# hpcaitech/CachedEmbedding

Measured on AMD Instinct MI355X. Metric: embedding lookups/sec (cache op + EmbeddingBag fwd + bwd/SGD), Criteo-1TB table @1% cache, higher is better.
Workload: dtype f32

## Files before the change

cachedembedding_amd/csrc/ce_bag.hip:

```cpp
#include <stdlib.h>

#include <algorithm>

#include "ce_common.h"

namespace ce {

#ifdef CE_ABLATIONS
#define CE_DBG(x) (x)
#else
#define CE_DBG(x) 0
#endif

struct BagParams {
  const float* weight;
  float* dst;
  const void* grad_out;
  const int64_t* indices;
  const void* offsets;
  const float* psw;
  int64_t nnz;
  int32_t num_bags;
  int32_t rowlen;
  int32_t g_log2;
// ... 305 lines not shown
  return lo;
}

template <typename KT> struct KeyOps;
template <> struct KeyOps<uint32_t> {
  static __device__ __forceinline__ uint32_t make(uint32_t row, int i) { return (row << 10) | (uint32_t)i; }
  static __device__ __forceinline__ uint32_t row(uint32_t k) { return k >> 10; }
  static __device__ __forceinline__ int idx(uint32_t k) { return (int)(k & 1023u); }
  static __device__ __forceinline__ uint32_t invalid() { return 0xffffffffu; }
  static __device__ __forceinline__ uint32_t row_invalid() { return 0x3fffffu; }
};
template <> struct KeyOps<unsigned long long> {
  static __device__ __forceinline__ unsigned long long make(uint32_t row, int i) {
    return ((unsigned long long)row << 32) | (uint32_t)i;
  }
  static __device__ __forceinline__ uint32_t row(unsigned long long k) { return (uint32_t)(k >> 32); }
  static __device__ __forceinline__ int idx(unsigned long long k) { return (int)(uint32_t)k; }
  static __device__ __forceinline__ unsigned long long invalid() { return ~0ull; }
  static __device__ __forceinline__ uint32_t row_invalid() { return 0xffffffffu; }
};

template <typename KT>
__device__ __forceinline__ KT shfl_xor_key(KT v, int m) { return __shfl_xor(v, m); }
template <>
__device__ __forceinline__ unsigned long long shfl_xor_key<unsigned long long>(unsigned long long v, int m) {
  const unsigned lo = __shfl_xor((unsigned)v, m), hi = __shfl_xor((unsigned)(v >> 32), m);
  return ((unsigned long long)hi << 32) | lo;
}

template <typename KT>
__device__ __forceinline__ void tile_sort_1024(KT (&key)[4], KT* lds, int tid) {
  for (int k = 2; k <= kBwdTile; k <<= 1) {
    for (int j = k >> 1; j > 0; j >>= 1) {
      if (j >= 256) {
#pragma unroll
        for (int r = 0; r < 4; ++r) lds[tid * 4 + r] = key[r];
        __syncthreads();
#pragma unroll
        for (int r = 0; r < 4; ++r) {
          const int i = tid * 4 + r;
          const KT other = lds[i ^ j];
          const bool lower = (i & j) == 0, up = (i & k) == 0;
          const KT lo = key[r] < other ? key[r] : other, hi = key[r] < other ? other : key[r];
          key[r] = (lower == up) ? lo : hi;
        }
        __syncthreads();
      } else if (j >= 4) {
#pragma unroll
        for (int r = 0; r < 4; ++r) {
          const int i = tid * 4 + r;
          const KT other = shfl_xor_key<KT>(key[r], j >> 2);
          const bool lower = (i & j) == 0, up = (i & k) == 0;
          const KT lo = key[r] < other ? key[r] : other, hi = key[r] < other ? other : key[r];
          key[r] = (lower == up) ? lo : hi;
        }
      } else {
#pragma unroll
        for (int r = 0; r < 4; ++r) {
          if (r & j) continue;
          const bool up = ((tid * 4 + r) & k) == 0;
          const KT a = key[r], b = key[r | j];
          if ((a > b) == up) {
            key[r] = b;
            key[r | j] = a;
          }
        }
      }
    }
  }
#pragma unroll
  for (int r = 0; r < 4; ++r) lds[tid * 4 + r] = key[r];
  __syncthreads();
}

constexpr int kSegLen = 16384;
constexpr int kSegKeys = 16;
#ifndef CE_SEG_BUCKETS
#define CE_SEG_BUCKETS 8192
#endif
constexpr int kSegBuckets = CE_SEG_BUCKETS;
constexpr int kExclRun = 32;
constexpr unsigned kExclFlag = 0x80000000u;

template <bool SRC, bool EXCL, bool ROWS>
__global__ __launch_bounds__(1024) void k_bag_presort_seg(const int64_t* __restrict__ indices, int64_t nnz_per_batch,
                                                         int32_t segs_per_batch, int64_t n_segs, uint32_t num_rows,
                                                         unsigned long long* __restrict__ keys_out, BagParams lay,
                                                         int64_t off_stride, const int64_t* __restrict__ ids,
                                                         int64_t* __restrict__ ids_minmax, int64_t* slots_io,
                                                         const int32_t* __restrict__ inverted,
                                                         const int* __restrict__ status) {
  __shared__ unsigned long long lk[kSegLen];
  static_assert(sizeof(unsigned long long) * kSegLen <= 160 * 1024 - 1024, "gfx950: 160 KB of LDS per CU");
  int* const cnt = (int*)lk;
  __shared__ int wsum[16];
  __shared__ long long mm_s[2][16];
  const int tid = threadIdx.x, lane = tid & 63, wv = tid >> 6;
  for (int64_t seg = blockIdx.x; seg < n_segs; seg += gridDim.x) {
    const int64_t batch = seg / segs_per_batch;
    const int sib = (int)(seg - batch * segs_per_batch);
    const int64_t in_base = batch * nnz_per_batch + (int64_t)sib * kSegLen;
    const int64_t base = seg * kSegLen;
    const int n_here = (int)min((int64_t)kSegLen, nnz_per_batch - (int64_t)sib * kSegLen);
    BagParams q = lay;
    if (SRC && lay.offsets) q.offsets = (const char*)lay.offsets + batch * off_stride * (lay.off64 ? 8 : 4);
    for (int i = tid; i <= kSegBuckets; i += 1024) cnt[i] = 0;
    __syncthreads();
    unsigned long long key[kSegKeys];
    int place[kSegKeys], bkt[kSegKeys];
    int32_t slot_r[ROWS ? kSegKeys : 1];
    if (ROWS) {
      const bool failed = *status != CE_OK;
      int32_t row_r[kSegKeys];
#pragma unroll
      for (int r = 0; r < kSegKeys; ++r) {
        const int e = r * 1024 + tid;
        row_r[r] = e < n_here ? (int32_t)slots_io[in_base + e] : -1;
      }
#pragma unroll
      for (int r = 0; r < kSegKeys; ++r) slot_r[r] = (row_r[r] >= 0 && !failed) ? inverted[row_r[r]] : -1;
#pragma unroll
      for (int r = 0; r < kSegKeys; ++r) {
        const int e = r * 1024 + tid;
        if (e < n_here) slots_io[in_base + e] = (int64_t)slot_r[r];
      }
    }
#pragma unroll
    for (int r = 0; r < kSegKeys; ++r) {
      const int e = r * 1024 + tid;
      key[r] = ~0ull;
      bkt[r] = kSegBuckets;
      if (e < n_here) {
        const int64_t row = ROWS ? (int64_t)slot_r[ROWS ? r : 0] : indices[in_base + e];
        const bool valid = (uint64_t)row < (uint64_t)num_rows;
        if (valid || SRC) {
          unsigned low = (unsigned)e;
          if (SRC && !(CE_DBG(lay.debug) & 2))
            low = (unsigned)out_row(q, lay.offsets ? find_bag(q, sib * kSegLen + e) : sib * kSegLen + e);
          key[r] = ((unsigned long long)(valid ? (uint32_t)row : 0xffffffffu) << 32) | low;
          if (valid) bkt[r] = (int)(row & (kSegBuckets - 1));
        }
      }
      if (CE_DBG(lay.debug) & 8) {
        place[r] = 0;
        continue;
      }
      const int b0 = __builtin_amdgcn_readfirstlane(bkt[r]);
      if (__all(bkt[r] == b0)) {
        int first = 0;
        if (lane == 0) first = atomicAdd(&cnt[b0], 64);
        place[r] = __shfl(first, 0) + lane;
      } else {
        place[r] = atomicAdd(&cnt[bkt[r]], 1);
      }
    }
    __syncthreads();
    constexpr int kPer = kSegBuckets / 1024;
    int c4[kPer], sum = 0;
#pragma unroll
    for (int q = 0; q < kPer; ++q) { c4[q] = cnt[tid * kPer + q]; sum += c4[q]; }
    int inc = sum;
#pragma unroll
    for (int d = 1; d < 64; d <<= 1) {
      const int o = __shfl_up(inc, d);
      if (lane >= d) inc += o;
    }
    if (lane == 63) wsum[wv] = inc;
    __syncthreads();
    int pre = inc - sum;
    for (int k = 0; k < wv; ++k) pre += wsum[k];
    int total = 0;
    for (int k = 0; k < 16; ++k) total += wsum[k];
#pragma unroll
    for (int q = 0; q < kPer; ++q) { cnt[tid * kPer + q] = pre; pre += c4[q]; }
    if (tid == 0) cnt[kSegBuckets] = total;
    __syncthreads();
    if (!EXCL) {
      int pos[kSegKeys];
#pragma unroll
      for (int r = 0; r < kSegKeys; ++r) pos[r] = cnt[bkt[r]] + place[r];
      __syncthreads();
#pragma unroll
      for (int r = 0; r < kSegKeys; ++r) lk[pos[r]] = key[r];
      __syncthreads();
#pragma unroll
      for (int r = 0; r < kSegKeys; ++r) keys_out[base + r * 1024 + tid] = lk[r * 1024 + tid];
      __syncthreads();
      continue;
    }
    int pos[kSegKeys];
#pragma unroll
    for (int r = 0; r < kSegKeys; ++r) pos[r] = cnt[bkt[r]] + place[r];
    __syncthreads();
#pragma unroll
    for (int r = 0; r < kSegKeys; ++r) lk[pos[r]] = key[r];
    __syncthreads();
    {
      const uint32_t* hi = (const uint32_t*)lk;
      const int p0 = tid * kSegKeys;
      for (int p = p0; p < p0 + kSegKeys; ++p) {
        const uint32_t row = hi[2 * p + 1];
        if (row == 0xffffffffu) break;
        const uint32_t b = row & (kSegBuckets - 1);
        if (p > 0 && (hi[2 * p - 1] & (kSegBuckets - 1)) == b && hi[2 * p - 1] != 0xffffffffu) continue;
        int e = p + 1;
        while (e < kSegLen && e - p <= kExclRun && hi[2 * e + 1] != 0xffffffffu && (hi[2 * e + 1] & (kSegBuckets - 1)) == b) ++e;
        if (e - p > kExclRun) continue;
        for (int i = p + 1; i < e; ++i) {
          const unsigned long long k = lk[i];
          int j = i;
          while (j > p && (uint32_t)(lk[j - 1] >> 32) > (uint32_t)(k >> 32)) { lk[j] = lk[j - 1]; --j; }
          lk[j] = k;
        }
        for (int a = p; a < e;) {
          int z = a + 1;
          while (z < e && (uint32_t)(lk[z] >> 32) == (uint32_t)(lk[a] >> 32)) ++z;
          if ((a >> 4) == ((z - 1) >> 4)) lk[a] |= kExclFlag;
          a = z;
        }
      }
    }
    __syncthreads();
#pragma unroll
    for (int r = 0; r < kSegKeys; ++r) keys_out[base + r * 1024 + tid] = lk[r * 1024 + tid];
    if (ids_minmax) {
      long long lo = INT64_MAX, hi2 = INT64_MIN;
      if (ids) {
#pragma unroll
        for (int r = 0; r < kSegKeys; ++r) {
          const int e = r * 1024 + tid;
          if (e < n_here) {
            const long long v = ids[in_base + e];
            lo = v < lo ? v : lo;
            hi2 = v > hi2 ? v : hi2;
          }
        }
      } else {
        lo = INT64_MIN; hi2 = INT64_MAX;
      }
#pragma unroll
      for (int d = 32; d >= 1; d >>= 1) {
        const long long ol = __shfl_xor(lo, d), oh = __shfl_xor(hi2, d);
        lo = ol < lo ? ol : lo;
        hi2 = oh > hi2 ? oh : hi2;
      }
      if (lane == 0) { mm_s[0][wv] = lo; mm_s[1][wv] = hi2; }
      __syncthreads();
      if (tid == 0) {
        for (int k = 1; k < 16; ++k) {
          lo = mm_s[0][k] < lo ? mm_s[0][k] : lo;
          hi2 = mm_s[1][k] > hi2 ? mm_s[1][k] : hi2;
        }
        ids_minmax[2 * seg] = lo;
        ids_minmax[2 * seg + 1] = hi2;
      }
    }
    __syncthreads();
  }
}

template <typename VT, int NCH, typename KT, int R, typename AT>
__global__ __launch_bounds__(256) void k_bag_bwd_tile(BagParams p) {
  using K = KeyOps<KT>;
  using A = Act<AT, VT>;
  __shared__ KT keys[kBwdTile];
  __shared__ int bagl[kBwdTile];
  __shared__ float scl[kBwdTile];

  const int tid = threadIdx.x;
  const int G = 1 << p.g_log2;
  const int ngroups = 256 >> p.g_log2;
  const int grp = tid >> p.g_log2;
  const int gl = tid & (G - 1);
  const int rowlen = p.rowlen;
  const int dim = rowlen * (int)(sizeof(VT) / 4);
  const typename A::V* __restrict__ GO = (const typename A::V*)p.grad_out;
  const int tile_len = p.tile_len;
  const int64_t total = p.presorted ? ((p.nnz + kSegLen - 1) / kSegLen) * kSegLen : p.nnz;
  const int ntiles = (int)((total + tile_len - 1) / tile_len);

  for (int tile = blockIdx.x; tile < ntiles; tile += gridDim.x) {
    const int j0 = tile * tile_len;
    const int nv = min(tile_len, (int)(total - j0));
    const bool presorted = p.presorted != nullptr;
    KT kr[4];
#pragma unroll
    for (int r = 0; r < 4; ++r) {
      const int i = tid * 4 + r;
      kr[r] = K::invalid();
      int j = j0 + i;
      uint32_t row = 0xffffffffu;
      if (presorted) {
        const unsigned long long sk = i < nv ? p.presorted[(int64_t)j0 + i] : ~0ull;
        j = -1;
        if (sk != ~0ull) {
          row = (uint32_t)(sk >> 32);
          j = (int)((((int64_t)j0 + i) / kSegLen) * kSegLen) + (int)(uint32_t)sk;
        }
      } else if (i < nv) {
        const int64_t r64 = p.indices[j];
        if ((uint64_t)r64 < (uint64_t)p.num_rows) row = (uint32_t)r64;
      } else {
        j = -1;
      }
      if (j >= 0) {
        const int bag = find_bag(p, j);
        float sc = p.alpha;
        if (p.psw) sc *= p.psw[j];
        if (p.mode == CE_MODE_MEAN) {
          const int len = bag_end(p, bag) - ld_off(p, bag);
          if (len > 1) sc = sc / (float)len;
        }
        bagl[i] = (int)out_row(p, bag);
        scl[i] = sc;
        if (row != 0xffffffffu) kr[r] = K::make(row, i);
      }
    }
    if (CE_DBG(p.debug) == 3) { __syncthreads(); continue; }
    if (presorted) {
#pragma unroll
      for (int r = 0; r < 4; ++r) keys[tid * 4 + r] = kr[r];
      __syncthreads();
    } else {
      tile_sort_1024<KT>(kr, keys, tid);
    }
    if (CE_DBG(p.debug) == 4) continue;
    const int kChunk = (nv + ngroups - 1) / ngroups;
    const int nchunks = (nv + kChunk - 1) / kChunk;
    for (int ck = grp; ck < nchunks; ck += ngroups) {
      const int s0 = ck * kChunk, s1 = min(nv, s0 + kChunk);
      VT acc[NCH];
#pragma unroll
      for (int c = 0; c < NCH; ++c) acc[c] = vzero<VT>();
      uint32_t cur = K::row(keys[s0]);
      for (int q = s0; q < s1; q += R) {
        VT v[R][NCH];
        float sc[R];
        uint32_t rw[R];
#pragma unroll
        for (int t = 0; t < R; ++t) {
          const KT key = (q + t < s1) ? keys[q + t] : K::invalid();
          const bool on = key != K::invalid();
          const int li = on ? K::idx(key) : 0;
          rw[t] = on ? K::row(key) : K::row_invalid();
          sc[t] = on ? scl[li] : 0.f;
          const int64_t orow = bagl[li];
#pragma unroll
          for (int c = 0; c < NCH; ++c) {
            const int ch = gl + c * G;
            v[t][c] = vzero<VT>();
            if (on && ch < rowlen) v[t][c] = A::up(__builtin_nontemporal_load(&GO[orow * rowlen + ch]));
          }
        }
        __builtin_amdgcn_s_waitcnt(0x0F70);
#pragma unroll
        for (int t = 0; t < R; ++t) {
          if (rw[t] != K::row_invalid()) {
            if (rw[t] != cur) {
#pragma unroll
              for (int c = 0; c < NCH; ++c) {
                if (cur != K::row_invalid())
                  flush_chunk(p.dst + (int64_t)cur * dim, acc[c], gl, G, c, rowlen, CE_DBG(p.debug));
                acc[c] = vzero<VT>();
              }
              cur = rw[t];
            }
#pragma unroll
            for (int c = 0; c < NCH; ++c) acc[c] = acc[c] + v[t][c] * sc[t];
          }
        }
      }
#pragma unroll
      for (int c = 0; c < NCH; ++c) {
        if (cur != K::row_invalid()) flush_chunk(p.dst + (int64_t)cur * dim, acc[c], gl, G, c, rowlen, CE_DBG(p.debug));
      }
    }
    __syncthreads();
  }
}

template <typename VT, int NCH, int R, bool NTG, bool EXCL, typename AT, bool PAIR = false>
__global__ __launch_bounds__(256) void k_bag_bwd_stream(BagParams p, int64_t total, const long long* __restrict__ seg_ranges) {
  using A = Act<AT, VT>;
  static_assert(!PAIR || (sizeof(typename A::V) == 8 && R % 2 == 0), "PAIR: 4 x 16 bit per lane, keys two at a time");
  __shared__ unsigned long long lk[256 * (R > 4 ? R : 4)];
  const int tid = threadIdx.x;
  const int G = 1 << p.g_log2;
  const int ngroups = 256 >> p.g_log2;
  const int grp = tid >> p.g_log2;
  const int gl = tid & (G - 1);
  const int rowlen = p.rowlen;
  const int dim = rowlen * (int)(sizeof(VT) / 4);
  const typename A::V* __restrict__ GO = (const typename A::V*)p.grad_out;
  const VT* __restrict__ WV = (const VT*)p.dst;
  const unsigned long long* __restrict__ keys = p.presorted;
  bool excl = false;
  if (EXCL) {
    const int nseg = (int)(total / kSegLen);
    int clash = nseg > 64 || seg_ranges == nullptr;
    if (!clash) {
      for (int pr = tid; pr < nseg * nseg; pr += 256) {
        const int a = pr / nseg, b2 = pr - a * nseg;
        if (a >= b2) continue;
        const long long alo = seg_ranges[2 * a], ahi = seg_ranges[2 * a + 1];
        const long long blo = seg_ranges[2 * b2], bhi = seg_ranges[2 * b2 + 1];
        if (alo <= ahi && blo <= bhi && !(ahi < blo || bhi < alo)) clash = 1;
      }
    }
    excl = __syncthreads_or(clash) == 0;
  }
  const int64_t all_groups = (int64_t)gridDim.x * ngroups;
  const int64_t round = R > 16 ? R : 16;
  const int64_t share = ((total + all_groups - 1) / all_groups + round - 1) / round * round;
  const int64_t s0 = share_of(p, grp, ngroups) * share;
  const int64_t s1 = min(total, s0 + share);
  if (s0 >= s1) return;
  const float alpha = p.alpha;
  const int kc = 4 * G > R ? 4 * G : R;
  unsigned long long* mylk = lk + grp * kc;
  VT acc[NCH];
#pragma unroll
  for (int c = 0; c < NCH; ++c) acc[c] = vzero<VT>();
  uint32_t cur = 0xffffffffu;
  bool cur_excl = false;
  for (int64_t c0 = s0; c0 < s1; c0 += kc) {
    for (int k = gl; k < kc; k += G) mylk[k] = c0 + k < s1 ? keys[c0 + k] : ~0ull;
    const int64_t c1 = min(s1, c0 + kc);
    for (int64_t q = c0; q < c1; q += R) {
      VT v[R][NCH];
      VT w2[EXCL ? R : 1][NCH];
      u32x4 raw[PAIR ? R / 2 : 1][NCH];
      uint32_t rw[R];
      uint32_t heads = 0;
#pragma unroll
      for (int t = 0; t < R; ++t) {
        const unsigned long long k = mylk[(int)(q - c0) + t];
        const bool on = k != ~0ull && (uint32_t)(k >> 32) < p.num_rows;
        rw[t] = on ? (uint32_t)(k >> 32) : 0xffffffffu;
        const uint32_t low = (uint32_t)k;
        const int64_t src = (int64_t)(low & ~kExclFlag);
        const bool head = EXCL && excl && on && (low & kExclFlag);
        if (head) heads |= 1u << t;
        if constexpr (PAIR) if (!(t & 1)) {
          const unsigned long long k1 = mylk[(int)(q - c0) + t + 1];
          const bool on1 = k1 != ~0ull && (uint32_t)(k1 >> 32) < p.num_rows;
          const bool mine = (gl & 1) ? on1 : on;
          const int64_t msrc = (gl & 1) ? (int64_t)((uint32_t)k1 & ~kExclFlag) : src;
#pragma unroll
          for (int c = 0; c < NCH; ++c) {
            const int ch = gl + c * G;
            raw[PAIR ? t / 2 : 0][c] = u32x4{0u, 0u, 0u, 0u};
            if (mine && ch < rowlen)
              raw[PAIR ? t / 2 : 0][c] = __builtin_nontemporal_load((const u32x4*)p.grad_out + ((msrc * rowlen + ch) >> 1));
          }
        }
#pragma unroll
        for (int c = 0; c < NCH; ++c) {
          const int ch = gl + c * G;
          v[t][c] = vzero<VT>();
          if (!PAIR && on && ch < rowlen)
            v[t][c] = A::up(NTG ? __builtin_nontemporal_load(&GO[src * rowlen + ch]) : GO[src * rowlen + ch]);
          if (EXCL) {
            w2[t][c] = vzero<VT>();
            if (head && ch < rowlen) w2[t][c] = WV[(int64_t)rw[t] * rowlen + ch];
          }
        }
      }
      __builtin_amdgcn_s_waitcnt(0x0F70);
      if constexpr (PAIR) {
#pragma unroll
        for (int t = 0; t < R; t += 2) {
#pragma unroll
          for (int c = 0; c < NCH; ++c) {
            const u32x4 r = raw[PAIR ? t / 2 : 0][c];
            const u32x2 lo{r.x, r.y}, hi{r.z, r.w};
            const bool odd = gl & 1;
            const u32x2 got = swap_with_pair(odd ? lo : hi);
            v[t][c] = A::up(__builtin_bit_cast(typename A::V, odd ? got : lo));
            v[t + 1][c] = A::up(__builtin_bit_cast(typename A::V, odd ? hi : got));
          }
        }
      }
#pragma unroll
      for (int t = 0; t < R; ++t) {
        if (rw[t] != 0xffffffffu) {
          const bool head = EXCL && ((heads >> t) & 1);
          if (rw[t] != cur || head) {
#pragma unroll
            for (int c = 0; c < NCH; ++c) {
              if (cur != 0xffffffffu) {
                if (EXCL && cur_excl) {
                  const int ch = gl + c * G;
                  if (ch < rowlen) ((VT*)(p.dst + (int64_t)cur * dim))[ch] = acc[c];
                } else {
                  flush_chunk(p.dst + (int64_t)cur * dim, acc[c], gl, G, c, rowlen, CE_DBG(p.debug));
                }
              }
              acc[c] = EXCL ? w2[EXCL ? t : 0][c] : vzero<VT>();
            }
            cur = rw[t];
            cur_excl = head;
          }
#pragma unroll
          for (int c = 0; c < NCH; ++c) acc[c] = acc[c] + v[t][c] * alpha;
        }
      }
    }
  }
  if (cur != 0xffffffffu) {
#pragma unroll
    for (int c = 0; c < NCH; ++c) {
      if (EXCL && cur_excl) {
        const int ch = gl + c * G;
        if (ch < rowlen) ((VT*)(p.dst + (int64_t)cur * dim))[ch] = acc[c];
      } else {
        flush_chunk(p.dst + (int64_t)cur * dim, acc[c], gl, G, c, rowlen, CE_DBG(p.debug));
      }
    }
  }
}

template <typename VT, int NCH, int R, int NTS, typename AT, bool PAIR = false>
__global__ __launch_bounds__(256, 4) void k_bag_fwd_keys(BagParams p, int64_t total) {
  using A = Act<AT, VT>;
  static_assert(!PAIR || (sizeof(typename A::V) == 8 && R % 2 == 0), "PAIR: 4 x 16 bit per lane, keys two at a time");
  __shared__ unsigned long long lk[256 * (R > 4 ? R : 4)];
  const int tid = threadIdx.x;
  const int G = 1 << p.g_log2;
  const int ngroups = 256 >> p.g_log2;
  const int grp = tid >> p.g_log2;
  const int gl = tid & (G - 1);
  const int rowlen = p.rowlen;
  const VT* __restrict__ W = (const VT*)p.weight;
  typename A::V* __restrict__ O = (typename A::V*)p.dst;
  const unsigned long long* __restrict__ keys = p.presorted;
  const int64_t all_groups = (int64_t)gridDim.x * ngroups;
  const int64_t round = R > 16 ? R : 16;
  const int64_t share = ((total + all_groups - 1) / all_groups + round - 1) / round * round;
  const int64_t s0 = share_of(p, grp, ngroups) * share;
  const int64_t s1 = min(total, s0 + share);
  if (s0 >= s1) return;
  const int kc = 4 * G > R ? 4 * G : R;
  unsigned long long* mylk = lk + grp * kc;
  VT prev[NCH];
#pragma unroll
  for (int c = 0; c < NCH; ++c) prev[c] = vzero<VT>();
  uint32_t prev_row = 0xffffffffu;
  for (int64_t c0 = s0; c0 < s1; c0 += kc) {
    for (int k = gl; k < kc; k += G) mylk[k] = c0 + k < s1 ? keys[c0 + k] : ~0ull;
    const int64_t c1 = min(s1, c0 + kc);
    for (int64_t q = c0; q < c1; q += R) {
      VT v[R][NCH];
      uint32_t heads = 0;
      uint32_t last = prev_row;
#pragma unroll
      for (int t = 0; t < R; ++t) {
        const unsigned long long k = mylk[(int)(q - c0) + t];
        const bool on = k != ~0ull;
        const uint32_t rw = (uint32_t)(k >> 32);
        const bool head = on && rw != last;
        if (on) last = rw;
        if (head) heads |= 1u << t;
#pragma unroll
        for (int c = 0; c < NCH; ++c) {
          const int ch = gl + c * G;
          v[t][c] = vzero<VT>();
          if (head && ch < rowlen && rw < p.num_rows) v[t][c] = W[(int64_t)rw * rowlen + ch];
        }
      }
      __builtin_amdgcn_s_waitcnt(0x0F70);
      if constexpr (PAIR) {
        const bool odd = gl & 1;
#pragma unroll
        for (int t = 0; t < R; t += 2) {
          const unsigned long long k0 = mylk[(int)(q - c0) + t], k1 = mylk[(int)(q - c0) + t + 1];
          if (k0 == ~0ull && k1 == ~0ull) continue;
          u32x2 r0[NCH], r1[NCH];
          if ((heads >> t) & 1) {
#pragma unroll
            for (int c = 0; c < NCH; ++c) prev[c] = v[t][c];
          }
#pragma unroll
          for (int c = 0; c < NCH; ++c) r0[c] = __builtin_bit_cast(u32x2, A::down(prev[c]));
          if ((heads >> (t + 1)) & 1) {
#pragma unroll
            for (int c = 0; c < NCH; ++c) prev[c] = v[t + 1][c];
          }
#pragma unroll
          for (int c = 0; c < NCH; ++c) r1[c] = __builtin_bit_cast(u32x2, A::down(prev[c]));
          const unsigned long long km = odd ? k1 : k0;
          const int64_t orow = (int64_t)((uint32_t)km & ~kExclFlag);
#pragma unroll
          for (int c = 0; c < NCH; ++c) {
            const int ch = gl + c * G;
            const u32x2 got = swap_with_pair(odd ? r0[c] : r1[c]);
            const u32x4 o = odd ? u32x4{got.x, got.y, r1[c].x, r1[c].y} : u32x4{r0[c].x, r0[c].y, got.x, got.y};
            if (km != ~0ull && ch < rowlen) store_out<NTS>((u32x4*)p.dst + ((orow * rowlen + ch) >> 1), o);
          }
        }
        prev_row = last;
        continue;
      }
#pragma unroll
      for (int t = 0; t < R; ++t) {
        const unsigned long long k = mylk[(int)(q - c0) + t];
        if (k == ~0ull) continue;
        if ((heads >> t) & 1) {
#pragma unroll
          for (int c = 0; c < NCH; ++c) prev[c] = v[t][c];
// ... 268 lines not shown
static int backward_sgd_impl(float* weight, int64_t num_rows, int32_t dim, const int64_t* indices, int64_t nnz,
                             const void* offsets, int32_t offsets_are_i64, int64_t num_bags,
                             int32_t include_last_offset, const float* per_sample_weights, int32_t mode,
                             int64_t hook_features, const void* grad_out, int act, float lr,
                             const unsigned long long* presorted, ce_stream_t stream) {
  CE_REQUIRE_ACT(act);
  if (num_bags == 0 || nnz == 0) return CE_OK;
  CE_REQUIRE(weight && grad_out && offsets && indices, CE_ERR_INVALID, "null pointer");
  BagParams p{};
  bool vec;
  int nch;
  int rc = fill_params(p, dim, indices, nnz, offsets, offsets_are_i64, num_bags, include_last_offset,
                       per_sample_weights, mode, hook_features, &vec, &nch, weight, act32(grad_out, act), nullptr,
                       act16(grad_out, act));
  if (rc) return rc;
  p.dst = weight;
  p.grad_out = grad_out;
  p.alpha = -lr;
  CE_REQUIRE(num_rows > 0 && num_rows < (int64_t)INT32_MAX, CE_ERR_INVALID, "num_rows out of range");
  p.num_rows = (uint32_t)num_rows;
  p.presorted = presorted;
  return launch_bwd_scatter(p, vec, nch, act, (hipStream_t)stream);
}

extern "C" int ce_bag_backward_sgd(float* weight, int64_t num_rows, int32_t dim, const int64_t* indices,
                                   int64_t nnz, const void* offsets, int32_t offsets_are_i64, int64_t num_bags,
                                   int32_t include_last_offset, const float* per_sample_weights, int32_t mode,
                                   int64_t hook_features, const float* grad_out, float lr, ce_stream_t stream) {
  return backward_sgd_impl(weight, num_rows, dim, indices, nnz, offsets, offsets_are_i64, num_bags,
                           include_last_offset, per_sample_weights, mode, hook_features, grad_out, CE_ACT_F32, lr, nullptr,
                           stream);
}

extern "C" int ce_bag_backward_sgd_act(float* weight, int64_t num_rows, int32_t dim, const int64_t* indices,
                                       int64_t nnz, const void* offsets, int32_t offsets_are_i64, int64_t num_bags,
                                       int32_t include_last_offset, const float* per_sample_weights, int32_t mode,
                                       int64_t hook_features, const void* grad_out, int32_t act_dtype, float lr,
                                       const uint64_t* presorted_keys, ce_stream_t stream) {
  return backward_sgd_impl(weight, num_rows, dim, indices, nnz, offsets, offsets_are_i64, num_bags,
                           include_last_offset, per_sample_weights, mode, hook_features, grad_out, act_dtype, lr,
                           (const unsigned long long*)presorted_keys, stream);
}

extern "C" int ce_bag_backward_sgd_presorted(float* weight, int64_t num_rows, int32_t dim, const int64_t* indices,
                                             int64_t nnz, const void* offsets, int32_t offsets_are_i64,
                                             int64_t num_bags, int32_t include_last_offset,
                                             const float* per_sample_weights, int32_t mode, int64_t hook_features,
                                             const float* grad_out, float lr, const uint64_t* presorted_keys,
                                             ce_stream_t stream) {
  CE_REQUIRE(presorted_keys, CE_ERR_INVALID, "null presorted_keys");
  return backward_sgd_impl(weight, num_rows, dim, indices, nnz, offsets, offsets_are_i64, num_bags,
                           include_last_offset, per_sample_weights, mode, hook_features, grad_out, CE_ACT_F32, lr,
                           (const unsigned long long*)presorted_keys, stream);
}

static int launch_bwd_stream(float* dst, int64_t num_rows, int32_t dim, int64_t nnz, const void* grad_out, int act,
                             float alpha, const unsigned long long* keys, const int64_t* seg_ranges, hipStream_t s) {
  CE_REQUIRE_ACT(act);
  if (nnz == 0) return CE_OK;
  CE_REQUIRE(dst && grad_out && keys, CE_ERR_INVALID, "null pointer");
  CE_REQUIRE(num_rows > 0 && num_rows < (int64_t)INT32_MAX, CE_ERR_INVALID, "num_rows out of range");
  BagParams p{};
  bool vec;
  int nch;
  int rc = fill_params(p, dim, nullptr, nnz, nullptr, 0, 0, 1, nullptr, CE_MODE_SUM, 0, &vec, &nch, dst,
                       act32(grad_out, act), nullptr, act16(grad_out, act));
  if (rc) return rc;
  p.dst = dst;
  p.grad_out = grad_out;
  p.alpha = alpha;
  p.num_rows = (uint32_t)num_rows;
  p.presorted = keys;
#ifdef CE_ABLATIONS
  { const char* dbg = getenv("CE_BWD_DEBUG"); p.debug = dbg ? atoi(dbg) : 0; }
#endif
  p.interleave = 1;
  const int64_t total = cdiv(nnz, kSegLen) * kSegLen;
  constexpr int per_cu = 6;
  const int ngroups = 256 >> p.g_log2;
  const int grid = (int)std::max<int64_t>(1, std::min<int64_t>((int64_t)kNumCU * per_cu, cdiv(total, (int64_t)ngroups * 16)));
  dim3 g(grid), b(256);
  const long long* rg = (const long long*)seg_ranges;
  const bool excl = seg_ranges != nullptr && vec && nch == 1;
#define CE_BWS(VT, N, R, EX) CE_ACT(act, hipLaunchKernelGGL((k_bag_bwd_stream<VT, N, R, true, EX, AT>), g, b, 0, s, p, total, rg))
#define CE_BWS2(N, R, EX)                                                                                              \
  do {                                                                                                                 \
    if (act == CE_ACT_BF16)                                                                                            \
      hipLaunchKernelGGL((k_bag_bwd_stream<f32x4, N, R, true, EX, bf16_t, true>), g, b, 0, s, p, total, rg);           \
    else                                                                                                               \
      hipLaunchKernelGGL((k_bag_bwd_stream<f32x4, N, R, true, EX, f16_t, true>), g, b, 0, s, p, total, rg);            \
  } while (0)
  if (vec && pair16(act, dim, grad_out)) {
    if (nch == 1 && excl) CE_BWS2(1, 16, true);
    else if (nch == 1) CE_BWS2(1, 16, false);
    else if (nch == 2) CE_BWS2(2, 8, false);
    else CE_BWS2(4, 4, false);
  } else if (vec) {
    if (nch == 1 && excl) CE_BWS(f32x4, 1, 16, true);
    else if (nch == 1) CE_BWS(f32x4, 1, 16, false);
    else if (nch == 2) CE_BWS(f32x4, 2, 8, false);
    else CE_BWS(f32x4, 4, 4, false);
  } else {
    if (nch == 1) CE_BWS(float, 1, 16, false);
    else if (nch == 2) CE_BWS(float, 2, 8, false);
    else CE_BWS(float, 4, 4, false);
  }
#undef CE_BWS
#undef CE_BWS2
  CE_LAUNCH_CHECK();
  return CE_OK;
}

extern "C" int ce_bag_backward_sgd_presorted_src(float* weight, int64_t num_rows, int32_t dim, int64_t nnz,
                                                 const float* grad_out, float lr, const uint64_t* src_keys,
                                                 ce_stream_t stream) {
  return launch_bwd_stream(weight, num_rows, dim, nnz, grad_out, CE_ACT_F32, -lr, (const unsigned long long*)src_keys,
                           nullptr, (hipStream_t)stream);
}

extern "C" int ce_bag_backward_sgd_presorted_src_excl(float* weight, int64_t num_rows, int32_t dim, int64_t nnz,
                                                      const float* grad_out, float lr, const uint64_t* src_keys,
                                                      const int64_t* seg_id_ranges, ce_stream_t stream) {
  return launch_bwd_stream(weight, num_rows, dim, nnz, grad_out, CE_ACT_F32, -lr, (const unsigned long long*)src_keys,
                           seg_id_ranges, (hipStream_t)stream);
}

extern "C" int ce_bag_backward_sgd_src_act(float* weight, int64_t num_rows, int32_t dim, int64_t nnz,
                                           const void* grad_out, int32_t act_dtype, float lr, const uint64_t* src_keys,
                                           const int64_t* seg_id_ranges, ce_stream_t stream) {
  return launch_bwd_stream(weight, num_rows, dim, nnz, grad_out, act_dtype, -lr, (const unsigned long long*)src_keys,
                           seg_id_ranges, (hipStream_t)stream);
}

extern "C" int ce_bag_backward_dense_src_act(float* grad_weight, int64_t num_rows, int32_t dim, int64_t nnz,
                                             const void* grad_out, int32_t act_dtype, const uint64_t* src_keys,
                                             ce_stream_t stream) {
  return launch_bwd_stream(grad_weight, num_rows, dim, nnz, grad_out, act_dtype, 1.f,
                           (const unsigned long long*)src_keys, nullptr, (hipStream_t)stream);
}

extern "C" int ce_bag_backward_dense_presorted_src(float* grad_weight, int64_t num_rows, int32_t dim, int64_t nnz,
                                                   const float* grad_out, const uint64_t* src_keys,
                                                   ce_stream_t stream) {
  return launch_bwd_stream(grad_weight, num_rows, dim, nnz, grad_out, CE_ACT_F32, 1.f,
                           (const unsigned long long*)src_keys, nullptr, (hipStream_t)stream);
}

extern "C" int ce_bag_forward_src_keys_act(const float* weight, int64_t num_rows, int32_t dim, int64_t nnz,
                                           const uint64_t* src_keys, void* out, int32_t act_dtype, ce_stream_t stream) {
  CE_REQUIRE_ACT(act_dtype);
  if (nnz == 0) return CE_OK;
  CE_REQUIRE(weight && src_keys && out, CE_ERR_INVALID, "null pointer");
  CE_REQUIRE(num_rows > 0 && num_rows < (int64_t)INT32_MAX, CE_ERR_INVALID, "num_rows out of range");
  BagParams p{};
  bool vec;
  int nch;
  int rc = fill_params(p, dim, nullptr, nnz, nullptr, 0, 0, 1, nullptr, CE_MODE_SUM, 0, &vec, &nch, weight,
                       act32(out, act_dtype), nullptr, act16(out, act_dtype));
  if (rc) return rc;
  p.weight = weight;
  p.dst = (float*)out;
  p.num_rows = (uint32_t)num_rows;
  p.presorted = (const unsigned long long*)src_keys;
  p.interleave = 0;
  const int64_t total = cdiv(nnz, kSegLen) * kSegLen;
  constexpr int per_cu = 16;
  const int ngroups = 256 >> p.g_log2;
  const int grid = (int)std::max<int64_t>(1, std::min<int64_t>((int64_t)kNumCU * per_cu, cdiv(total, (int64_t)ngroups * 16)));
  dim3 g(grid), b(256);
  hipStream_t s = (hipStream_t)stream;
#define CE_FWK(VT, N, R) CE_ACT(act_dtype, hipLaunchKernelGGL((k_bag_fwd_keys<VT, N, R, 1, AT>), g, b, 0, s, p, total))
#define CE_FWK2(N, R)                                                                                     \
  do {                                                                                                    \
    if (act_dtype == CE_ACT_BF16)                                                                         \
      hipLaunchKernelGGL((k_bag_fwd_keys<f32x4, N, R, 1, bf16_t, true>), g, b, 0, s, p, total);           \
    else                                                                                                  \
      hipLaunchKernelGGL((k_bag_fwd_keys<f32x4, N, R, 1, f16_t, true>), g, b, 0, s, p, total);            \
  } while (0)
  if (vec && pair16(act_dtype, dim, out)) {
    if (nch == 1) CE_FWK2(1, 16);
    else if (nch == 2) CE_FWK2(2, 8); else CE_FWK2(4, 4);
  } else if (vec) {
    if (nch == 1) CE_FWK(f32x4, 1, 16);
    else if (nch == 2) CE_FWK(f32x4, 2, 8); else CE_FWK(f32x4, 4, 4);
  } else {
    if (nch == 1) CE_FWK(float, 1, 16); else if (nch == 2) CE_FWK(float, 2, 8); else CE_FWK(float, 4, 4);
  }
#undef CE_FWK
#undef CE_FWK2
  CE_LAUNCH_CHECK();
  return CE_OK;
}

extern "C" int ce_bag_forward_src_keys(const float* weight, int64_t num_rows, int32_t dim, int64_t nnz,
                                       const uint64_t* src_keys, float* out, ce_stream_t stream) {
  return ce_bag_forward_src_keys_act(weight, num_rows, dim, nnz, src_keys, out, CE_ACT_F32, stream);
}

extern "C" int64_t ce_bag_presort_len(int64_t nnz) { return nnz <= 0 ? 0 : cdiv(nnz, kSegLen) * kSegLen; }

static int presort_window_impl(const int64_t* indices, int64_t nnz_per_batch, int64_t n_batches, int64_t num_rows,
                               uint64_t* keys_out, const BagParams* lay, int64_t off_stride, const int64_t* ids,
                               int64_t* ids_minmax, ce_stream_t stream) {
  if (nnz_per_batch == 0 || n_batches == 0) return CE_OK;
  CE_REQUIRE(indices && keys_out && nnz_per_batch > 0 && n_batches > 0, CE_ERR_INVALID, "bad arguments");
  CE_REQUIRE(nnz_per_batch < (int64_t)INT32_MAX - kSegLen, CE_ERR_INVALID, "batch too large");
  CE_REQUIRE(num_rows > 0 && num_rows < (int64_t)INT32_MAX, CE_ERR_INVALID, "num_rows out of range");
  const int64_t spb = cdiv(nnz_per_batch, kSegLen);
  const int64_t nseg = spb * n_batches;
  CE_REQUIRE(spb < (int64_t)INT32_MAX && nseg < (int64_t)INT32_MAX, CE_ERR_INVALID, "too many segments");
  const dim3 grid((unsigned)std::min<int64_t>(nseg, kMaxBlocks)), block(1024);
  int64_t* const no_io = nullptr;
  const int32_t* const no_inv = nullptr;
  const int* const no_st = nullptr;
  if (lay && ids_minmax)
    hipLaunchKernelGGL((k_bag_presort_seg<true, true, false>), grid, block, 0, (hipStream_t)stream, indices, nnz_per_batch,
                       (int32_t)spb, nseg, (uint32_t)num_rows, (unsigned long long*)keys_out, *lay, off_stride, ids,
                       ids_minmax, no_io, no_inv, no_st);
  else if (lay)
    hipLaunchKernelGGL((k_bag_presort_seg<true, false, false>), grid, block, 0, (hipStream_t)stream, indices, nnz_per_batch,
                       (int32_t)spb, nseg, (uint32_t)num_rows, (unsigned long long*)keys_out, *lay, off_stride,
                       (const int64_t*)nullptr, (int64_t*)nullptr, no_io, no_inv, no_st);
  else
    hipLaunchKernelGGL((k_bag_presort_seg<false, false, false>), grid, block, 0, (hipStream_t)stream, indices, nnz_per_batch,
                       (int32_t)spb, nseg, (uint32_t)num_rows, (unsigned long long*)keys_out, BagParams{}, 0ll,
                       (const int64_t*)nullptr, (int64_t*)nullptr, no_io, no_inv, no_st);
  CE_LAUNCH_CHECK();
  return CE_OK;
}

namespace ce {
int presort_window_from_rows(int64_t* slots_io, int64_t nnz_per_batch, int64_t n_batches, int64_t num_rows,
                             const int32_t* inverted, const int* status, int32_t src_keys, const void* offsets,
                             int32_t offsets_are_i64, int64_t offsets_batch_stride, int64_t num_bags,
                             int32_t include_last_offset, int64_t hook_features, uint64_t* keys_out, hipStream_t stream) {
  if (nnz_per_batch == 0 || n_batches == 0) return CE_OK;
  CE_REQUIRE(slots_io && keys_out && inverted && status && nnz_per_batch > 0 && n_batches > 0, CE_ERR_INVALID, "bad arguments");
  CE_REQUIRE(nnz_per_batch < (int64_t)INT32_MAX - kSegLen, CE_ERR_INVALID, "batch too large");
  CE_REQUIRE(num_rows > 0 && num_rows < (int64_t)INT32_MAX, CE_ERR_INVALID, "num_rows out of range");
  const int64_t spb = cdiv(nnz_per_batch, kSegLen);
  const int64_t nseg = spb * n_batches;
  CE_REQUIRE(spb < (int64_t)INT32_MAX && nseg < (int64_t)INT32_MAX, CE_ERR_INVALID, "too many segments");
  const dim3 grid((unsigned)std::min<int64_t>(nseg, kMaxBlocks)), block(1024);
  if (src_keys) {
    CE_REQUIRE(num_bags > 0 && offsets_batch_stride >= 0, CE_ERR_INVALID, "bad offsets");
    CE_REQUIRE(offsets || num_bags == nnz_per_batch, CE_ERR_INVALID,
               "offsets may only be NULL for the one-id-per-bag layout (num_bags == nnz_per_batch)");
    BagParams lay{};
    bool vec;
    int nch;
    int rc = fill_params(lay, 4, nullptr, nnz_per_batch, offsets, offsets_are_i64, num_bags, include_last_offset, nullptr,
                         CE_MODE_SUM, hook_features, &vec, &nch, nullptr, nullptr, nullptr);
    if (rc) return rc;
    hipLaunchKernelGGL((k_bag_presort_seg<true, false, true>), grid, block, 0, stream, (const int64_t*)nullptr,
                       nnz_per_batch, (int32_t)spb, nseg, (uint32_t)num_rows, (unsigned long long*)keys_out, lay,
                       offsets_batch_stride, (const int64_t*)nullptr, (int64_t*)nullptr, slots_io, inverted, status);
  } else {
    hipLaunchKernelGGL((k_bag_presort_seg<false, false, true>), grid, block, 0, stream, (const int64_t*)nullptr,
                       nnz_per_batch, (int32_t)spb, nseg, (uint32_t)num_rows, (unsigned long long*)keys_out, BagParams{},
                       0ll, (const int64_t*)nullptr, (int64_t*)nullptr, slots_io, inverted, status);
  }
  CE_LAUNCH_CHECK();
  return CE_OK;
}
}

extern "C" int ce_bag_presort_window(const int64_t* indices, int64_t nnz_per_batch, int64_t n_batches,
                                     int64_t num_rows, uint64_t* keys_out, ce_stream_t stream) {
  return presort_window_impl(indices, nnz_per_batch, n_batches, num_rows, keys_out, nullptr, 0, nullptr, nullptr, stream);
}

static int presort_window_src_impl(const int64_t* indices, int64_t nnz_per_batch, int64_t n_batches, int64_t num_rows,
                                   const void* offsets, int32_t offsets_are_i64, int64_t offsets_batch_stride,
                                   int64_t num_bags, int32_t include_last_offset, int64_t hook_features,
                                   const int64_t* ids, uint64_t* keys_out, int64_t* seg_id_ranges, ce_stream_t stream) {
  if (nnz_per_batch == 0 || n_batches == 0) return CE_OK;
  CE_REQUIRE(num_bags > 0 && offsets_batch_stride >= 0, CE_ERR_INVALID, "bad offsets");
  CE_REQUIRE(offsets || num_bags == nnz_per_batch, CE_ERR_INVALID,
             "offsets may only be NULL for the one-id-per-bag layout (num_bags == nnz_per_batch)");
  BagParams lay{};
  bool vec;
  int nch;
  int rc = fill_params(lay, 4, indices, nnz_per_batch, offsets, offsets_are_i64, num_bags, include_last_offset,
                       nullptr, CE_MODE_SUM, hook_features, &vec, &nch, nullptr, nullptr, nullptr);
  if (rc) return rc;
#ifdef CE_ABLATIONS
  { const char* dbg = getenv("CE_PRESORT_DEBUG"); lay.debug = dbg ? atoi(dbg) : 0; }
#endif
  return presort_window_impl(indices, nnz_per_batch, n_batches, num_rows, keys_out, &lay, offsets_batch_stride, ids,
                             seg_id_ranges, stream);
}

extern "C" int ce_bag_presort_window_src(const int64_t* indices, int64_t nnz_per_batch, int64_t n_batches,
                                         int64_t num_rows, const void* offsets, int32_t offsets_are_i64,
                                         int64_t offsets_batch_stride, int64_t num_bags, int32_t include_last_offset,
                                         int64_t hook_features, uint64_t* keys_out, ce_stream_t stream) {
  return presort_window_src_impl(indices, nnz_per_batch, n_batches, num_rows, offsets, offsets_are_i64,
                                 offsets_batch_stride, num_bags, include_last_offset, hook_features, nullptr, keys_out,
                                 nullptr, stream);
}

extern "C" int ce_bag_presort_window_src_excl(const int64_t* indices, int64_t nnz_per_batch, int64_t n_batches,
                                              int64_t num_rows, const void* offsets, int32_t offsets_are_i64,
                                              int64_t offsets_batch_stride, int64_t num_bags,
                                              int32_t include_last_offset, int64_t hook_features, const int64_t* ids,
                                              uint64_t* keys_out, int64_t* seg_id_ranges, ce_stream_t stream) {
  CE_REQUIRE(seg_id_ranges, CE_ERR_INVALID, "null seg_id_ranges");
  return presort_window_src_impl(indices, nnz_per_batch, n_batches, num_rows, offsets, offsets_are_i64,
                                 offsets_batch_stride, num_bags, include_last_offset, hook_features, ids, keys_out,
                                 seg_id_ranges, stream);
}

extern "C" int ce_bag_presort(const int64_t* indices, int64_t nnz, int64_t num_rows, uint64_t* keys_out,
                              ce_stream_t stream) {
  return ce_bag_presort_window(indices, nnz, 1, num_rows, keys_out, stream);
}

extern "C" int ce_rows_axpy(float* weight, int64_t num_rows, int32_t dim, const int64_t* index, int64_t n,
                            const float* src_rows, float alpha, ce_stream_t stream) {
  if (n == 0) return CE_OK;
  CE_REQUIRE(weight && index && src_rows, CE_ERR_INVALID, "null pointer");
  CE_REQUIRE(dim > 0 && n > 0 && n < (int64_t)INT32_MAX, CE_ERR_INVALID, "bad sizes");
  CE_REQUIRE(num_rows > 0 && num_rows < (int64_t)INT32_MAX, CE_ERR_INVALID, "num_rows out of range");
  auto al16 = [](const void* q) { return (((uintptr_t)q) & 15) == 0; };
  const bool vec = (dim % 4 == 0) && al16(weight) && al16(src_rows);
  const int rowlen = vec ? dim / 4 : dim;
  int g = 1, gl2 = 0;
  while (g < rowlen && g < 64) { g <<= 1; ++gl2; }
  const int need = (rowlen + g - 1) / g;
  int nch = 1;
  while (nch < need) nch <<= 1;
  CE_REQUIRE(nch <= 4, CE_ERR_UNSUPPORTED, "embedding dim %d too large for this build", dim);
  const int u = nch == 1 ? 8 : (nch == 2 ? 4 : 2);
  const int64_t per_block = (int64_t)(64 / g) * u * 4;
  dim3 grid(grid_for(n, (int)per_block)), block(256);
  hipStream_t s = (hipStream_t)stream;
#define CE_AXPY(VT, N)                                                                                      \
  hipLaunchKernelGGL((k_rows_axpy<VT, N>), grid, block, 0, s, weight, (uint32_t)num_rows, index, n,         \
                     (const VT*)src_rows, rowlen, gl2, dim, alpha)
  if (vec) {
    if (nch == 1) CE_AXPY(f32x4, 1); else if (nch == 2) CE_AXPY(f32x4, 2); else CE_AXPY(f32x4, 4);
  } else {
    if (nch == 1) CE_AXPY(float, 1); else if (nch == 2) CE_AXPY(float, 2); else CE_AXPY(float, 4);
// ... 24 lines not shown
```

Baseline: 3.273 billion.

## Replace LDS-staged segment presort with two-sweep count/scatter kernel; size key LDS dynamically

After: 3.241 billion. Within noise of the previous version (-1.0%).

```diff
diff --git a/cachedembedding_amd/csrc/ce_bag.hip b/cachedembedding_amd/csrc/ce_bag.hip
--- a/cachedembedding_amd/csrc/ce_bag.hip
+++ b/cachedembedding_amd/csrc/ce_bag.hip
@@ -411,14 +411,38 @@
 constexpr int kExclRun = 32;
 constexpr unsigned kExclFlag = 0x80000000u;
 
-template <bool SRC, bool EXCL, bool ROWS>
+__device__ __forceinline__ void seg_scan_counters(int* cnt, int* wsum, int tid) {
+  const int lane = tid & 63, wv = tid >> 6;
+  __syncthreads();
+  constexpr int kPer = kSegBuckets / 1024;
+  int c4[kPer], sum = 0;
+#pragma unroll
+  for (int q = 0; q < kPer; ++q) { c4[q] = cnt[tid * kPer + q]; sum += c4[q]; }
+  int inc = sum;
+#pragma unroll
+  for (int d = 1; d < 64; d <<= 1) {
+    const int o = __shfl_up(inc, d);
+    if (lane >= d) inc += o;
+  }
+  if (lane == 63) wsum[wv] = inc;
+  __syncthreads();
+  int pre = inc - sum;
+  for (int k = 0; k < wv; ++k) pre += wsum[k];
+  int total = 0;
+  for (int k = 0; k < 16; ++k) total += wsum[k];
+#pragma unroll
+  for (int q = 0; q < kPer; ++q) { cnt[tid * kPer + q] = pre; pre += c4[q]; }
+  if (tid == 0) cnt[kSegBuckets] = total;
+  __syncthreads();
+}
+
+template <bool SRC, bool EXCL>
 __global__ __launch_bounds__(1024) void k_bag_presort_seg(const int64_t* __restrict__ indices, int64_t nnz_per_batch,
                                                          int32_t segs_per_batch, int64_t n_segs, uint32_t num_rows,
                                                          unsigned long long* __restrict__ keys_out, BagParams lay,
                                                          int64_t off_stride, const int64_t* __restrict__ ids,
-                                                         int64_t* __restrict__ ids_minmax, int64_t* slots_io,
-                                                         const int32_t* __restrict__ inverted,
-                                                         const int* __restrict__ status) {
+                                                         int64_t* __restrict__ ids_minmax) {
+  static_assert(SRC && EXCL, "the forms without owner-exclusive runs are k_bag_presort_2sweep");
   __shared__ unsigned long long lk[kSegLen];
   static_assert(sizeof(unsigned long long) * kSegLen <= 160 * 1024 - 1024, "gfx950: 160 KB of LDS per CU");
   int* const cnt = (int*)lk;
@@ -437,30 +461,13 @@
     __syncthreads();
     unsigned long long key[kSegKeys];
     int place[kSegKeys], bkt[kSegKeys];
-    int32_t slot_r[ROWS ? kSegKeys : 1];
-    if (ROWS) {
-      const bool failed = *status != CE_OK;
-      int32_t row_r[kSegKeys];
-#pragma unroll
-      for (int r = 0; r < kSegKeys; ++r) {
-        const int e = r * 1024 + tid;
-        row_r[r] = e < n_here ? (int32_t)slots_io[in_base + e] : -1;
-      }
-#pragma unroll
-      for (int r = 0; r < kSegKeys; ++r) slot_r[r] = (row_r[r] >= 0 && !failed) ? inverted[row_r[r]] : -1;
-#pragma unroll
-      for (int r = 0; r < kSegKeys; ++r) {
-        const int e = r * 1024 + tid;
-        if (e < n_here) slots_io[in_base + e] = (int64_t)slot_r[r];
-      }
-    }
 #pragma unroll
     for (int r = 0; r < kSegKeys; ++r) {
       const int e = r * 1024 + tid;
       key[r] = ~0ull;
       bkt[r] = kSegBuckets;
       if (e < n_here) {
-        const int64_t row = ROWS ? (int64_t)slot_r[ROWS ? r : 0] : indices[in_base + e];
+        const int64_t row = indices[in_base + e];
         const bool valid = (uint64_t)row < (uint64_t)num_rows;
         if (valid || SRC) {
           unsigned low = (unsigned)e;
@@ -483,40 +490,7 @@
         place[r] = atomicAdd(&cnt[bkt[r]], 1);
       }
     }
-    __syncthreads();
-    constexpr int kPer = kSegBuckets / 1024;
-    int c4[kPer], sum = 0;
-#pragma unroll
-    for (int q = 0; q < kPer; ++q) { c4[q] = cnt[tid * kPer + q]; sum += c4[q]; }
-    int inc = sum;
-#pragma unroll
-    for (int d = 1; d < 64; d <<= 1) {
-      const int o = __shfl_up(inc, d);
-      if (lane >= d) inc += o;
-    }
-    if (lane == 63) wsum[wv] = inc;
-    __syncthreads();
-    int pre = inc - sum;
-    for (int k = 0; k < wv; ++k) pre += wsum[k];
-    int total = 0;
-    for (int k = 0; k < 16; ++k) total += wsum[k];
-#pragma unroll
-    for (int q = 0; q < kPer; ++q) { cnt[tid * kPer + q] = pre; pre += c4[q]; }
-    if (tid == 0) cnt[kSegBuckets] = total;
-    __syncthreads();
-    if (!EXCL) {
-      int pos[kSegKeys];
-#pragma unroll
-      for (int r = 0; r < kSegKeys; ++r) pos[r] = cnt[bkt[r]] + place[r];
-      __syncthreads();
-#pragma unroll
-      for (int r = 0; r < kSegKeys; ++r) lk[pos[r]] = key[r];
-      __syncthreads();
-#pragma unroll
-      for (int r = 0; r < kSegKeys; ++r) keys_out[base + r * 1024 + tid] = lk[r * 1024 + tid];
-      __syncthreads();
-      continue;
-    }
+    seg_scan_counters(cnt, wsum, tid);
     int pos[kSegKeys];
 #pragma unroll
     for (int r = 0; r < kSegKeys; ++r) pos[r] = cnt[bkt[r]] + place[r];
@@ -588,6 +562,97 @@
   }
 }
 
+constexpr int kSweep = 4;
+template <bool SRC, bool ROWS>
+__global__ __launch_bounds__(1024) __attribute__((amdgpu_waves_per_eu(7))) void k_bag_presort_2sweep(const int64_t* __restrict__ indices, int64_t nnz_per_batch,
+                                                            int32_t segs_per_batch, int64_t n_segs, uint32_t num_rows,
+                                                            unsigned long long* __restrict__ keys_out, BagParams lay,
+                                                            int64_t off_stride, int64_t* slots_io,
+                                                            const int32_t* __restrict__ inverted,
+                                                            const int* __restrict__ status) {
+  __shared__ int cnt[kSegBuckets + 1];
+  __shared__ int wsum[16];
+  static_assert(kSegKeys % kSweep == 0, "whole sweeps");
+  const int tid = threadIdx.x, lane = tid & 63;
+  const int64_t* const src = ROWS ? slots_io : indices;
+  for (int64_t seg = blockIdx.x; seg < n_segs; seg += gridDim.x) {
+    const int64_t batch = seg / segs_per_batch;
+    const int sib = (int)(seg - batch * segs_per_batch);
+    const int64_t in_base = batch * nnz_per_batch + (int64_t)sib * kSegLen;
+    const int64_t base = seg * kSegLen;
+    const int n_here = (int)min((int64_t)kSegLen, nnz_per_batch - (int64_t)sib * kSegLen);
+    BagParams q = lay;
+    if (SRC && lay.offsets) q.offsets = (const char*)lay.offsets + batch * off_stride * (lay.off64 ? 8 : 4);
+    for (int i = tid; i <= kSegBuckets; i += 1024) cnt[i] = 0;
+    __syncthreads();
+    const bool failed = ROWS && *status != CE_OK;
+    for (int r0 = 0; r0 < kSegKeys; r0 += kSweep) {
+      uint32_t row[kSweep];
+#pragma unroll
+      for (int u = 0; u < kSweep; ++u) {
+        const int e = (r0 + u) * 1024 + tid;
+        const int64_t v = e < n_here ? src[in_base + e] : -1;
+        row[u] = ROWS ? (uint32_t)v : ((uint64_t)v < (uint64_t)num_rows ? (uint32_t)v : 0xffffffffu);
+      }
+      if (ROWS) {
+        int32_t slot[kSweep];
+#pragma unroll
+        for (int u = 0; u < kSweep; ++u) slot[u] = ((int32_t)row[u] >= 0 && !failed) ? inverted[(int32_t)row[u]] : -1;
+#pragma unroll
+        for (int u = 0; u < kSweep; ++u) {
+          const int e = (r0 + u) * 1024 + tid;
+          if (e < n_here) slots_io[in_base + e] = (int64_t)slot[u];
+          row[u] = (uint32_t)slot[u] < num_rows ? (uint32_t)slot[u] : 0xffffffffu;
+        }
+      }
+#pragma unroll
+      for (int u = 0; u < kSweep; ++u) {
+        const int bkt = row[u] != 0xffffffffu ? (int)(row[u] & (kSegBuckets - 1)) : kSegBuckets;
+        const int b0 = __builtin_amdgcn_readfirstlane(bkt);
+        if (__all(bkt == b0)) {
+          if (lane == 0) atomicAdd(&cnt[b0], 64);
+        } else {
+          atomicAdd(&cnt[bkt], 1);
+        }
+      }
+    }
+    seg_scan_counters(cnt, wsum, tid);
+    for (int r0 = 0; r0 < kSegKeys; r0 += kSweep) {
+      uint32_t row[kSweep];
+#pragma unroll
+      for (int u = 0; u < kSweep; ++u) {
+        const int e = (r0 + u) * 1024 + tid;
+        const int64_t v = e < n_here ? src[in_base + e] : -1;
+        row[u] = (uint64_t)v < (uint64_t)num_rows ? (uint32_t)v : 0xffffffffu;
+      }
+#pragma unroll
+      for (int u = 0; u < kSweep; ++u) {
+        const int e = (r0 + u) * 1024 + tid;
+        const bool valid = row[u] != 0xffffffffu;
+        unsigned long long key = ~0ull;
+        if (e < n_here && (valid || SRC)) {
+          unsigned low = (unsigned)e;
+          if (SRC && !(CE_DBG(lay.debug) & 2))
+            low = (unsigned)out_row(q, lay.offsets ? find_bag(q, sib * kSegLen + e) : sib * kSegLen + e);
+          key = ((unsigned long long)row[u] << 32) | low;
+        }
+        const int bkt = valid ? (int)(row[u] & (kSegBuckets - 1)) : kSegBuckets;
+        int pos;
+        const int b0 = __builtin_amdgcn_readfirstlane(bkt);
+        if (__all(bkt == b0)) {
+          int first = 0;
+          if (lane == 0) first = atomicAdd(&cnt[b0], 64);
+          pos = __shfl(first, 0) + lane;
+        } else {
+          pos = atomicAdd(&cnt[bkt], 1);
+        }
+        keys_out[base + pos] = key;
+      }
+    }
+    __syncthreads();
+  }
+}
+
 template <typename VT, int NCH, typename KT, int R, typename AT>
 __global__ __launch_bounds__(256) void k_bag_bwd_tile(BagParams p) {
   using K = KeyOps<KT>;
@@ -708,11 +773,16 @@
   }
 }
 
+static inline unsigned key_slice_bytes(int g_log2, int R) {
+  const int G = 1 << g_log2, kc = 4 * G > R ? 4 * G : R;
+  return (unsigned)((256 >> g_log2) * kc * sizeof(unsigned long long));
+}
+
 template <typename VT, int NCH, int R, bool NTG, bool EXCL, typename AT, bool PAIR = false>
 __global__ __launch_bounds__(256) void k_bag_bwd_stream(BagParams p, int64_t total, const long long* __restrict__ seg_ranges) {
   using A = Act<AT, VT>;
   static_assert(!PAIR || (sizeof(typename A::V) == 8 && R % 2 == 0), "PAIR: 4 x 16 bit per lane, keys two at a time");
-  __shared__ unsigned long long lk[256 * (R > 4 ? R : 4)];
+  extern __shared__ unsigned long long lk[];
   const int tid = threadIdx.x;
   const int G = 1 << p.g_log2;
   const int ngroups = 256 >> p.g_log2;
@@ -853,7 +923,7 @@
 __global__ __launch_bounds__(256, 4) void k_bag_fwd_keys(BagParams p, int64_t total) {
   using A = Act<AT, VT>;
   static_assert(!PAIR || (sizeof(typename A::V) == 8 && R % 2 == 0), "PAIR: 4 x 16 bit per lane, keys two at a time");
-  __shared__ unsigned long long lk[256 * (R > 4 ? R : 4)];
+  extern __shared__ unsigned long long lk[];
   const int tid = threadIdx.x;
   const int G = 1 << p.g_log2;
   const int ngroups = 256 >> p.g_log2;
@@ -1288,13 +1358,14 @@
   dim3 g(grid), b(256);
   const long long* rg = (const long long*)seg_ranges;
   const bool excl = seg_ranges != nullptr && vec && nch == 1;
-#define CE_BWS(VT, N, R, EX) CE_ACT(act, hipLaunchKernelGGL((k_bag_bwd_stream<VT, N, R, true, EX, AT>), g, b, 0, s, p, total, rg))
+#define CE_BWS(VT, N, R, EX) \
+  CE_ACT(act, hipLaunchKernelGGL((k_bag_bwd_stream<VT, N, R, true, EX, AT>), g, b, key_slice_bytes(p.g_log2, R), s, p, total, rg))
 #define CE_BWS2(N, R, EX)                                                                                              \
   do {                                                                                                                 \
     if (act == CE_ACT_BF16)                                                                                            \
-      hipLaunchKernelGGL((k_bag_bwd_stream<f32x4, N, R, true, EX, bf16_t, true>), g, b, 0, s, p, total, rg);           \
+      hipLaunchKernelGGL((k_bag_bwd_stream<f32x4, N, R, true, EX, bf16_t, true>), g, b, key_slice_bytes(p.g_log2, R), s, p, total, rg); \
     else                                                                                                               \
-      hipLaunchKernelGGL((k_bag_bwd_stream<f32x4, N, R, true, EX, f16_t, true>), g, b, 0, s, p, total, rg);            \
+      hipLaunchKernelGGL((k_bag_bwd_stream<f32x4, N, R, true, EX, f16_t, true>), g, b, key_slice_bytes(p.g_log2, R), s, p, total, rg); \
   } while (0)
   if (vec && pair16(act, dim, grad_out)) {
     if (nch == 1 && excl) CE_BWS2(1, 16, true);
@@ -1375,13 +1446,14 @@
   const int grid = (int)std::max<int64_t>(1, std::min<int64_t>((int64_t)kNumCU * per_cu, cdiv(total, (int64_t)ngroups * 16)));
   dim3 g(grid), b(256);
   hipStream_t s = (hipStream_t)stream;
-#define CE_FWK(VT, N, R) CE_ACT(act_dtype, hipLaunchKernelGGL((k_bag_fwd_keys<VT, N, R, 1, AT>), g, b, 0, s, p, total))
+#define CE_FWK(VT, N, R) \
+  CE_ACT(act_dtype, hipLaunchKernelGGL((k_bag_fwd_keys<VT, N, R, 1, AT>), g, b, key_slice_bytes(p.g_log2, R), s, p, total))
 #define CE_FWK2(N, R)                                                                                     \
   do {                                                                                                    \
     if (act_dtype == CE_ACT_BF16)                                                                         \
-      hipLaunchKernelGGL((k_bag_fwd_keys<f32x4, N, R, 1, bf16_t, true>), g, b, 0, s, p, total);           \
+      hipLaunchKernelGGL((k_bag_fwd_keys<f32x4, N, R, 1, bf16_t, true>), g, b, key_slice_bytes(p.g_log2, R), s, p, total); \
     else                                                                                                  \
-      hipLaunchKernelGGL((k_bag_fwd_keys<f32x4, N, R, 1, f16_t, true>), g, b, 0, s, p, total);            \
+      hipLaunchKernelGGL((k_bag_fwd_keys<f32x4, N, R, 1, f16_t, true>), g, b, key_slice_bytes(p.g_log2, R), s, p, total); \
   } while (0)
   if (vec && pair16(act_dtype, dim, out)) {
     if (nch == 1) CE_FWK2(1, 16);
@@ -1420,17 +1492,17 @@
   const int32_t* const no_inv = nullptr;
   const int* const no_st = nullptr;
   if (lay && ids_minmax)
-    hipLaunchKernelGGL((k_bag_presort_seg<true, true, false>), grid, block, 0, (hipStream_t)stream, indices, nnz_per_batch,
+    hipLaunchKernelGGL((k_bag_presort_seg<true, true>), grid, block, 0, (hipStream_t)stream, indices, nnz_per_batch,
                        (int32_t)spb, nseg, (uint32_t)num_rows, (unsigned long long*)keys_out, *lay, off_stride, ids,
-                       ids_minmax, no_io, no_inv, no_st);
+                       ids_minmax);
   else if (lay)
-    hipLaunchKernelGGL((k_bag_presort_seg<true, false, false>), grid, block, 0, (hipStream_t)stream, indices, nnz_per_batch,
-                       (int32_t)spb, nseg, (uint32_t)num_rows, (unsigned long long*)keys_out, *lay, off_stride,
-                       (const int64_t*)nullptr, (int64_t*)nullptr, no_io, no_inv, no_st);
+    hipLaunchKernelGGL((k_bag_presort_2sweep<true, false>), grid, block, 0, (hipStream_t)stream, indices, nnz_per_batch,
+                       (int32_t)spb, nseg, (uint32_t)num_rows, (unsigned long long*)keys_out, *lay, off_stride, no_io,
+                       no_inv, no_st);
   else
-    hipLaunchKernelGGL((k_bag_presort_seg<false, false, false>), grid, block, 0, (hipStream_t)stream, indices, nnz_per_batch,
-                       (int32_t)spb, nseg, (uint32_t)num_rows, (unsigned long long*)keys_out, BagParams{}, 0ll,
-                       (const int64_t*)nullptr, (int64_t*)nullptr, no_io, no_inv, no_st);
+    hipLaunchKernelGGL((k_bag_presort_2sweep<false, false>), grid, block, 0, (hipStream_t)stream, indices, nnz_per_batch,
+                       (int32_t)spb, nseg, (uint32_t)num_rows, (unsigned long long*)keys_out, BagParams{}, 0ll, no_io,
+                       no_inv, no_st);
   CE_LAUNCH_CHECK();
   return CE_OK;
 }
@@ -1458,13 +1530,13 @@
     int rc = fill_params(lay, 4, nullptr, nnz_per_batch, offsets, offsets_are_i64, num_bags, include_last_offset, nullptr,
                          CE_MODE_SUM, hook_features, &vec, &nch, nullptr, nullptr, nullptr);
     if (rc) return rc;
-    hipLaunchKernelGGL((k_bag_presort_seg<true, false, true>), grid, block, 0, stream, (const int64_t*)nullptr,
+    hipLaunchKernelGGL((k_bag_presort_2sweep<true, true>), grid, block, 0, stream, (const int64_t*)nullptr,
                        nnz_per_batch, (int32_t)spb, nseg, (uint32_t)num_rows, (unsigned long long*)keys_out, lay,
-                       offsets_batch_stride, (const int64_t*)nullptr, (int64_t*)nullptr, slots_io, inverted, status);
+                       offsets_batch_stride, slots_io, inverted, status);
   } else {
-    hipLaunchKernelGGL((k_bag_presort_seg<false, false, true>), grid, block, 0, stream, (const int64_t*)nullptr,
+    hipLaunchKernelGGL((k_bag_presort_2sweep<false, true>), grid, block, 0, stream, (const int64_t*)nullptr,
                        nnz_per_batch, (int32_t)spb, nseg, (uint32_t)num_rows, (unsigned long long*)keys_out, BagParams{},
-                       0ll, (const int64_t*)nullptr, (int64_t*)nullptr, slots_io, inverted, status);
+                       0ll, slots_io, inverted, status);
   }
   CE_LAUNCH_CHECK();
   return CE_OK;
```
